# zcash/halo2

Hardware: AMD Instinct MI355X
Metric: Pallas MSM Mscalar-mults/s (+ Fp NTT Gbutterflies/s) at k=20 (higher is better)
Workload: dtype u256 (8x32-bit Montgomery limbs)

## Files before the change

__graft_entry__.py:

```python
import os
import subprocess
import sys

ROOT = os.path.dirname(os.path.abspath(__file__))
if ROOT not in sys.path:
    sys.path.insert(0, ROOT)


def build() -> None:
    subprocess.check_call(["make", "-C", os.path.join(ROOT, "halo2_amd", "csrc"), "-j8", "all", "ab"])
    subprocess.check_call(["make", "-C", os.path.join(ROOT, "oracle")])
    os.makedirs(os.path.join(ROOT, "build"), exist_ok=True)
    subprocess.check_call(["/opt/rocm/bin/hipcc", "--offload-arch=gfx950", "-O3",
                           os.path.join(ROOT, "tests", "native", "field_check.hip"), os.path.join(ROOT, "oracle", "h2_oracle.c"),
                           "-o", os.path.join(ROOT, "build", "field_check")], stderr=subprocess.DEVNULL)
    subprocess.check_call(["/opt/rocm/bin/hipcc", "--offload-arch=gfx950", "-O3",
                           os.path.join(ROOT, "tests", "native", "h2c_edge_driver.hip"), "-o", os.path.join(ROOT, "build", "h2c_edge_driver")])
    subprocess.check_call(["/opt/rocm/bin/hipcc", "--offload-arch=gfx950", "-O3",
                           os.path.join(ROOT, "tests", "native", "field_edge_driver.hip"), "-o", os.path.join(ROOT, "build", "field_edge_driver")])
    subprocess.check_call(["g++", "-O2", "-std=c++17", os.path.join(ROOT, "tests", "native", "host_mirror_check.cpp"),
                           "-L" + os.path.join(ROOT, "halo2_amd"), "-lhalo2_mi355x", "-L" + os.path.join(ROOT, "oracle"), "-lh2oracle",
                           "-Wl,-rpath,$ORIGIN/../halo2_amd", "-Wl,-rpath,$ORIGIN/../oracle", "-lpthread", "-lm",
                           "-o", os.path.join(ROOT, "build", "host_mirror_check")])
    subprocess.check_call(["g++", "-O2", "-std=c++17", os.path.join(ROOT, "tests", "native", "modinv_check.cpp"), "-o", os.path.join(ROOT, "build", "modinv_check")])
    hb = subprocess.run(["/opt/rocm/bin/hipcc", "-O2", "-std=c++17", os.path.join(ROOT, "bench", "native", "h2bench.cpp"),
                         "-L" + os.path.join(ROOT, "oracle"), "-lh2oracle", "-Wl,-rpath,$ORIGIN/../oracle", "-ldl", "-lpthread",
                         "-o", os.path.join(ROOT, "build", "h2bench")], stdout=subprocess.DEVNULL, stderr=subprocess.PIPE, text=True)
    if hb.returncode != 0:
        print("warning: bench/native/h2bench.cpp did not build (the library and the tests do not need it):\n" + hb.stderr[-2000:], file=sys.stderr)
    import halo2_amd
    halo2_amd.lib()


def smoke() -> None:
    import numpy as np

    import halo2_amd as h
    from halo2_amd import fields
    from oracle import c_oracle as co
    from oracle import pasta

    assert h.lib().h2_init(0) == 0, h.lib().h2_last_error()
    curve, n = h.PALLAS, 1 << 12
    sf = co.field_of_curve(curve, "scalar")
    scal = co.random_field(sf, 1, n)
    bases = co.generate_bases(curve, 2, n)
    got = h.best_multiexp(scal, bases, curve)
    want = co.best_multiexp(curve, scal, bases)
    assert co.jac_to_affine_ints(curve, got) == co.jac_to_affine_ints(curve, want), "MSM parity"
    log_n = 12
    a = co.random_field(h.FP, 3, 1 << log_n)
    omega = fields.scalar_limbs(pasta.omega_for(pasta.P, log_n), h.FP)
    assert np.array_equal(h.best_fft(a.copy(), omega, log_n, h.FP), co.best_fft(h.FP, a, omega, log_n)), "NTT parity"
    params = h.Params.new(h.VESTA, 5)
    vs = co.field_of_curve(h.VESTA, "scalar")
    got_w = co.jac_to_affine_ints(h.VESTA, params.commit_lagrange(np.zeros((32, 4), dtype=np.uint64), h.Blind(field=vs)))
    assert got_w == (0x2bbc94ef7b22aebef24f9a4b0cc1831882548b605171366017d45c3e6fd92075,
                     0x082b801a6e176239943bfb759fb02138f47a5c8cc4aa7fa0af559fde4e3abd97), "reference-pinned commitment"
    params.close()
    print("smoke ok: 2^12 Pallas MSM and 2^12 Fp NTT bit-exact vs oracle; Params.new(5) commits to the reference-pinned point")


if __name__ == "__main__":
    build()
    if len(sys.argv) > 1 and sys.argv[1] == "smoke":
        smoke()
```

halo2_amd/csrc/msm_fold.hip:

```cpp
#include "msm_internal.cuh"

namespace h2 {

static_assert(r256_tree_bytes(kTreeLanes) == (kTreeLanes / kGroup) * 128, "a quad of lanes per point of the 8 x 32 tree");

template <int FB>
__global__ void __launch_bounds__(256) msm_finish_buckets(const u32 *__restrict__ heads, const u32 *__restrict__ starts,
                                                          u32 *__restrict__ buckets, u32 *__restrict__ heavy,
                                                          u32 total_buckets, u32 T, u32 div) {
    H2_LATENCY_STAGE();
    const u32 b = (blockIdx.x * blockDim.x + threadIdx.x) / kGroup;
    if (b >= total_buckets) return;
    const bool lead = (threadIdx.x & (kGroup - 1)) == 0;
    const HeadRange h = bucket_heads<false>(starts, b, total_buckets, T, div);
    if (h.h1 <= h.h0) return;
    if (h.h1 - h.h0 > kHeavy && heavy_park<kGroup>(heavy, b, lead)) return;
    xyzz<FB> acc = xyzz_load<FB>(buckets + 32 * (size_t)b);
    xyzz<FB> nxt = xyzz_load<FB>(heads + 32 * (size_t)h.h0);
    for (u32 t = h.h0; t < h.h1; ++t) {
        xyzz<FB> p = nxt;
        if (t + 1 < h.h1) nxt = xyzz_load<FB>(heads + 32 * (size_t)(t + 1));
        xyzz_add_wide<FB>(acc, p);
    }
    if (lead) xyzz_store<FB>(buckets + 32 * (size_t)b, acc);
}
template <int FB>
__global__ void __launch_bounds__(256) msm_finish_heavy(const u32 *__restrict__ heads, const u32 *__restrict__ starts,
                                                        u32 *__restrict__ scratch, const u32 *__restrict__ heavy,
                                                        u32 total_buckets, u32 T, u32 div) {
    H2_LATENCY_STAGE();
    extern __shared__ __attribute__((aligned(16))) u32 sh[];
    if (blockIdx.y >= min(heavy[1], kMaxHeavy)) return;
    const HeadRange h = bucket_heads<false>(starts, heavy[2 + blockIdx.y], total_buckets, T, div);
    const u32 share = (h.h1 - h.h0 + kHeavyBlocks - 1) / kHeavyBlocks;
    const u32 lo = h.h0 + blockIdx.x * share, hi = min(h.h1, lo + share);
    const xyzz<FB> acc = r256_quad_gather<FB>(heads, hi > lo ? hi - lo : 0u, [lo](u32 k) { return lo + k; });
    r256_quads_sum<FB>(acc, sh, blockDim.x / kGroup);
    if (threadIdx.x == 0) {
        xyzz<FB> r = xyzz_load<FB>(sh);
        xyzz_store<FB>(scratch + 32 * ((size_t)blockIdx.y * kHeavyBlocks + blockIdx.x), r);
    }
}
template <int FB>
__global__ void __launch_bounds__(64) msm_finish_heavy2(const u32 *__restrict__ scratch, u32 *__restrict__ buckets,
                                                        const u32 *__restrict__ heavy) {
    H2_LATENCY_STAGE();
    __shared__ __attribute__((aligned(16))) u32 sh[32 * 16];
    if (blockIdx.x >= min(heavy[1], kMaxHeavy)) return;
    const u32 b = heavy[2 + blockIdx.x], q = threadIdx.x / kGroup;
    const bool lead = (threadIdx.x & (kGroup - 1)) == 0;
    const u32 *src = scratch + 32 * ((size_t)blockIdx.x * kHeavyBlocks);
    xyzz<FB> acc = xyzz_load<FB>(src + 32 * q);
    for (u32 i = q + 16; i < kHeavyBlocks; i += 16) {
        xyzz<FB> p = xyzz_load<FB>(src + 32 * i);
        xyzz_add_wide<FB>(acc, p);
    }
    r256_quads_sum<FB>(acc, sh, 16);
    if (q == 0) {
        xyzz<FB> r = xyzz_load<FB>(sh), own = xyzz_load<FB>(buckets + 32 * (size_t)b);
        xyzz_add_wide<FB>(r, own);
        if (lead) xyzz_store<FB>(buckets + 32 * (size_t)b, r);
    }
}

template <int FB>
__global__ void __launch_bounds__(256) msm_bucket_add(u32 *__restrict__ total, const u32 *__restrict__ part, u32 nb) {
    H2_LATENCY_STAGE();
    const u32 b = (blockIdx.x * blockDim.x + threadIdx.x) / kGroup;
    if (b >= nb) return;
    const xyzz<FB> p = xyzz_load<FB>(part + 32 * (size_t)b);
    if (fe_is_zero(p.zz)) return;
    xyzz<FB> acc = xyzz_load<FB>(total + 32 * (size_t)b);
    xyzz_add_wide<FB>(acc, p);
    if ((threadIdx.x & (kGroup - 1)) == 0) xyzz_store<FB>(total + 32 * (size_t)b, acc);
}

template <int FB>
__global__ void __launch_bounds__(256) fold9_finish(const u32 *__restrict__ heads9, const u32 *__restrict__ starts, u32 *__restrict__ buckets9,
                                                    u32 *__restrict__ heavy, u32 total_buckets, u32 T, u32 div, ColStride cs) {
    fold9_stage(cs);
    const u32 b = blockIdx.x * blockDim.x + threadIdx.x;
    if (b >= total_buckets) return;
    if (gridDim.z > 1) {
        heads9 = H2_COLZ(heads9, cs.heads);
        starts = H2_COLZ(starts, cs.starts);
        buckets9 = H2_COLZ(buckets9, cs.buckets);
        heavy = H2_COLZ(heavy, cs.heavy);
    }
    const HeadRange h = bucket_heads<true>(starts, b, total_buckets, T, div);
    if (h.h1 <= h.h0) return;
    if (h.h1 - h.h0 > kHeavy && heavy_park<1>(heavy, b, true)) return;
    xyzz9<FB> acc = xyzz9_load_raw<FB>(buckets9 + 36 * (size_t)b);
    for (u32 t = h.h0; t < h.h1; ++t) xyzz9_add<FB>(acc, xyzz9_load_raw<FB>(heads9 + 36 * (size_t)t));
    xyzz9_store_raw<FB>(buckets9 + 36 * (size_t)b, acc);
}
template <int FB>
__global__ void __launch_bounds__(256, 3) fold9_finish_heavy(const u32 *__restrict__ heads9, const u32 *__restrict__ starts, u32 *__restrict__ scratch9,
                                                          const u32 *__restrict__ heavy, u32 total_buckets, u32 T, u32 div, ColStride cs) {
    fold9_stage(cs);
    __shared__ __attribute__((aligned(16))) u32 sh[32 * 36];
    if (gridDim.z > 1) {
        heavy = H2_COLZ(heavy, cs.heavy);
        heads9 = H2_COLZ(heads9, cs.heads);
        starts = H2_COLZ(starts, cs.starts);
        scratch9 = H2_COLZ(scratch9, cs.hscratch);
    }
    const u32 count = min(heavy[1], kMaxHeavy);
    const HeadSplit hs = head_split<true>(starts, total_buckets, T, div);
    for (u32 slot = blockIdx.y; slot < count; slot += gridDim.y) {
        const HeadRange h = bucket_heads(hs, starts, heavy[2 + slot]);
        const u32 share = (h.h1 - h.h0 + kHeavyBlocks - 1) / kHeavyBlocks;
        const u32 lo = h.h0 + blockIdx.x * share, hi = min(h.h1, lo + share);
        xyzz9<FB> acc = fold9_quad_gather<FB, H2_FOLD_D>(heads9, hi > lo ? hi - lo : 0u, [lo](u32 k) { return lo + k; });
        acc = fold9_quads_sum<FB>(acc, sh);
        if (fold9_root() && (threadIdx.x & (kGroup - 1)) == 0) xyzz9_store_raw<FB>(scratch9 + 36 * ((size_t)slot * kHeavyBlocks + blockIdx.x), acc);
        __syncthreads();
    }
}
template <int FB>
__global__ void __launch_bounds__(64, 3) fold9_finish_heavy2(const u32 *__restrict__ scratch9, u32 *__restrict__ buckets9, const u32 *__restrict__ heavy,
                                                             ColStride cs) {
    fold9_stage(cs);
    __shared__ __attribute__((aligned(16))) u32 sh[8 * 36];
    if (gridDim.z > 1) {
        heavy = H2_COLZ(heavy, cs.heavy);
        scratch9 = H2_COLZ(scratch9, cs.hscratch);
        buckets9 = H2_COLZ(buckets9, cs.buckets);
    }
    const u32 count = min(heavy[1], kMaxHeavy);
    for (u32 slot = blockIdx.x; slot < count; slot += gridDim.x) {
        const u32 b = heavy[2 + slot];
        const u32 *src = scratch9 + 36 * ((size_t)slot * kHeavyBlocks);
        xyzz9<FB> acc = fold9_quad_gather<FB, H2_FOLD_D>(src, kHeavyBlocks, [](u32 k) { return k; });
        acc = fold9_quads_sum<FB>(acc, sh);
        if (fold9_root()) {
            xyzz9_add_wide<FB>(acc, xyzz9_load_raw<FB>(buckets9 + 36 * (size_t)b));
            if ((threadIdx.x & (kGroup - 1)) == 0) xyzz9_store_raw<FB>(buckets9 + 36 * (size_t)b, acc);
        }
        __syncthreads();
    }
}
template <int FB>
__global__ void __launch_bounds__(256, 3) fold9_rowcol(const u32 *__restrict__ buckets9, u32 *__restrict__ lines9, u32 S, u32 NR, ColStride cs) {
    fold9_stage(cs);
    __shared__ __attribute__((aligned(16))) u32 sh[32 * 36];
    if (gridDim.z > 1) {
        buckets9 = H2_COLZ(buckets9, cs.buckets);
        lines9 = H2_COLZ(lines9, cs.lines);
    }
    const bool is_col = blockIdx.x < S;
    const u32 id = is_col ? blockIdx.x : blockIdx.x - S + 1;
    const u32 cnt = is_col ? NR : S;
    const u32 base = blockIdx.y * S * NR + (is_col ? id : id * S), step = is_col ? S : 1;
    xyzz9<FB> acc = fold9_quad_gather<FB, H2_FOLD_D>(buckets9, cnt, [base, step](u32 k) { return base + k * step; });
    acc = fold9_quads_sum<FB>(acc, sh);
    if (fold9_root() && (threadIdx.x & (kGroup - 1)) == 0)
        xyzz9_store_raw<FB>(lines9 + 36 * ((size_t)blockIdx.y * (S + NR) + (is_col ? id : S + id)), acc);
}
template <int FB>
__global__ void __launch_bounds__(256, 3) fold9_planes(const u32 *__restrict__ lines9, u32 *__restrict__ planes9, u32 *__restrict__ counter, u32 S, u32 NR,
                                                    int cb, u32 *__restrict__ out, int out_kind, int out_mont, ColOut co, ColStride cs) {
    fold9_stage(cs);
    __shared__ __attribute__((aligned(16))) u32 sh[32 * 36];
    __shared__ u32 s_last;
    if (gridDim.z > 1) {
        lines9 = H2_COLZ(lines9, cs.lines);
        planes9 = H2_COLZ(planes9, cs.planes);
        counter = H2_COLZ(counter, cs.ctr);
        out = co.out[blockIdx.z];
    }
    const u32 t = blockIdx.x, planes = gridDim.x;
    lines9 += 36 * (size_t)blockIdx.y * (S + NR);
    planes9 += 36 * (size_t)blockIdx.y * 32;
    counter += blockIdx.y;
    out += (out_kind == kOutSliceSum ? 32 : point_out_words(out_kind)) * (size_t)blockIdx.y;
    xyzz9<FB> acc = fold9_quad_gather<FB, H2_FOLD_D>(lines9, fold9_plane_cols(S, cb, t) + fold9_plane_rows(NR, cb, t),
                                                     [=](u32 k) { return fold9_plane_line(S, cb, t, k); });
    acc = fold9_quads_sum<FB>(acc, sh);
    if (!fold9_plane_arrive<FB>(acc, t, planes9, counter, planes, s_last)) return;
    acc = fold9_quad_gather<FB, H2_FOLD_D>(planes9, planes, [](u32 k) { return k; });
    acc = fold9_quads_sum<FB>(acc, sh);
    if (!fold9_root()) return;
    const xyzz<FB> r = xyzz9_to_r256_wide<FB>(acc);
    if ((threadIdx.x & (kGroup - 1)) != 0) return;
    *counter = 0;
    if (out_kind == kOutSliceSum) {
        xyzz_store<FB>(out, r);
        return;
    }
    point_out_store<FB>(out, r, out_kind, out_mont);
}


template <int FB>
__global__ void __launch_bounds__(256) msm_reduce_segments(const u32 *__restrict__ buckets, u32 *__restrict__ partial,
                                                           u32 NB, u32 total_segments, int seg) {
    H2_LATENCY_STAGE();
    const u32 t = (blockIdx.x * blockDim.x + threadIdx.x) / kGroup;
    if (t >= total_segments) return;
    u32 segs_per_slice = NB / seg;
    u32 sl = t / segs_per_slice, sg = t % segs_per_slice;
    const u32 *base = buckets + 32 * ((size_t)sl * NB + (size_t)sg * seg);
    xyzz<FB> run = xyzz_identity<FB>(), acc = xyzz_identity<FB>();
    for (int j = seg - 1; j >= 0; --j) {
        xyzz<FB> bk = xyzz_load<FB>(base + 32 * j);
        xyzz_add_wide<FB>(run, bk);
        xyzz_add_wide<FB>(acc, run);
    }
    xyzz<FB> sh = xyzz_mul_small_wide<FB>(run, sg * seg);
    xyzz_add_wide<FB>(acc, sh);
    if ((threadIdx.x & (kGroup - 1)) == 0) xyzz_store<FB>(partial + 32 * (size_t)t, acc);
}

template <int FB>
__global__ void __launch_bounds__(256) msm_sum_slice(const u32 *__restrict__ partial, u32 *__restrict__ out, u32 per_slice,
                                                     u32 share) {
    H2_LATENCY_STAGE();
    extern __shared__ __attribute__((aligned(16))) u32 sh[];
    const u32 sl = blockIdx.y, blk = blockIdx.x;
    const u32 lo = blk * share, hi = min(per_slice, lo + share);
    const xyzz<FB> acc = r256_quad_gather<FB>(partial + 32 * (size_t)sl * per_slice, hi > lo ? hi - lo : 0u, [lo](u32 k) { return lo + k; });
    r256_quads_sum<FB>(acc, sh, blockDim.x / kGroup);
    if (threadIdx.x == 0) {
        xyzz<FB> r = xyzz_load<FB>(sh);
        xyzz_store<FB>(out + 32 * ((size_t)sl * gridDim.x + blk), r);
    }
}

template <int FB>
__global__ void __launch_bounds__(256) msm_rowcol_sums(const u32 *__restrict__ buckets, u32 *__restrict__ wide, u32 S, u32 NR) {
    H2_LATENCY_STAGE();
    extern __shared__ __attribute__((aligned(16))) u32 sh[];
    const bool is_col = blockIdx.x < S;
    const u32 id = is_col ? blockIdx.x : blockIdx.x - S + 1;
    const size_t base = is_col ? id : (size_t)id * S, step = is_col ? S : 1;
    const xyzz<FB> acc = r256_quad_gather<FB>(buckets, is_col ? NR : S, [base, step](u32 k) { return base + (size_t)k * step; });
    r256_quads_sum<FB>(acc, sh, blockDim.x / kGroup);
    if (threadIdx.x == 0) {
        xyzz<FB> r = xyzz_load<FB>(sh);
        xyzz_store<FB>(wide + 32 * (is_col ? (size_t)id : (size_t)NR + id - 1), r);
    }
}

template <int FB>
__global__ void __launch_bounds__(64) msm_combine(const u32 *__restrict__ slice_sums, int slices, int c, u32 *__restrict__ out,
                                                  int out_kind, int out_mont, int extra_dbl, const u32 *__restrict__ addend, int addend_first) {
    H2_LATENCY_STAGE();
    if (threadIdx.x >= kGroup) return;
    if (gridDim.x > 1) {
        slice_sums += 32 * (size_t)blockIdx.x;
        out += point_out_words(out_kind) * (size_t)blockIdx.x;
        slices = 1;
    }
    xyzz9<FB> r9 = xyzz9_identity<FB>();
    for (int w = slices - 1; w >= 0; --w) {
        if (w != slices - 1)
            for (int k = 0; k < c; ++k) r9 = xyzz9_dbl_wide<FB>(r9);
        const xyzz9<FB> s9 = xyzz9_from_r256_wide<FB>(xyzz_load<FB>(slice_sums + 32 * (size_t)w));
        xyzz9_add_wide<FB>(r9, s9);
    }
    if (addend && addend_first) xyzz9_add_wide<FB>(r9, xyzz9_from_r256_wide<FB>(xyzz_load<FB>(addend)));
    for (int k = 0; k < extra_dbl; ++k) r9 = xyzz9_dbl_wide<FB>(r9);
    if (addend && !addend_first) xyzz9_add_wide<FB>(r9, xyzz9_from_r256_wide<FB>(xyzz_load<FB>(addend)));
    const xyzz<FB> r = xyzz9_to_r256_wide<FB>(r9);
    if (threadIdx.x != 0) return;
    if (out_kind == kOutSliceSum) {
        xyzz_store<FB>(out, r);
        return;
    }
    point_out_store<FB>(out, r, out_kind, out_mont);
}

template <int FB>
__global__ void __launch_bounds__(64) msm_combine_ranges(RangeSums rs, int ranges, int slices, int c, u32 *__restrict__ out, int out_kind, int out_mont) {
    H2_LATENCY_STAGE();
    __shared__ __attribute__((aligned(16))) u32 sh[16 * 36];
    const int w = threadIdx.x / kGroup;
    const bool lead = (threadIdx.x & (kGroup - 1)) == 0;
    if (w < slices) {
        xyzz9<FB> acc = xyzz9_identity<FB>();
        for (int q = 0; q < ranges; ++q) xyzz9_add_wide<FB>(acc, xyzz9_from_r256_wide<FB>(xyzz_load<FB>(rs.p[q] + 32 * (size_t)w)));
        if (lead) xyzz9_store_raw<FB>(sh + 36 * w, acc);
    }
    __syncthreads();
    if (threadIdx.x >= kGroup) return;
    xyzz9<FB> r9 = xyzz9_identity<FB>();
    for (int s = slices - 1; s >= 0; --s) {
        if (s != slices - 1)
            for (int k = 0; k < c; ++k) r9 = xyzz9_dbl_wide<FB>(r9);
        xyzz9_add_wide<FB>(r9, xyzz9_load_raw<FB>(sh + 36 * s));
    }
    const xyzz<FB> r = xyzz9_to_r256_wide<FB>(r9);
    if (threadIdx.x == 0) point_out_store<FB>(out, r, out_kind, out_mont);
}

#define H2_FOLD_FB(fb, f, ...) ((fb) == FP ? f<FP>(__VA_ARGS__) : f<FQ>(__VA_ARGS__))

template <int FB> static void fold9_group_launch(hipStream_t st, const Fold9Group &g) {
    const ColStride &cs = g.cs;
    const u32 fz = cs.joined ? 1 : g.cols, ftb = cs.joined ? g.cols * g.tb : g.tb;
    const u32 S = g.wideS, NR = g.wideNR;
    u32 *lines = g.lines9 + 36 * (size_t)g.slice0 * (S + NR);
    hipLaunchKernelGGL((fold9_finish<FB>), dim3((ftb + 255) / 256, 1, fz), dim3(256), 0, st, g.heads9, g.starts, g.buckets9, g.heavy, ftb, g.T, g.lane_div, cs);
    hipLaunchKernelGGL((fold9_finish_heavy<FB>), dim3(kHeavyBlocks, kHeavyRows, fz), dim3(256), 0, st, g.heads9, g.starts, g.hscratch, (const u32 *)g.heavy, ftb, g.T, g.lane_div, cs);
    hipLaunchKernelGGL((fold9_finish_heavy2<FB>), dim3(kHeavyRows, 1, fz), dim3(64), 0, st, (const u32 *)g.hscratch, g.buckets9, (const u32 *)g.heavy, cs);
    hipLaunchKernelGGL((fold9_rowcol<FB>), dim3(S + NR - 1, g.nslices, g.cols), dim3(256), 0, st, (const u32 *)g.buckets9, lines, S, NR, cs);
    hipLaunchKernelGGL((fold9_planes<FB>), dim3(fold9_plane_count(g.c), g.nslices, g.cols), dim3(256), 0, st, (const u32 *)lines, g.planes9 + 36 * (size_t)g.slice0 * 32, g.ctr + g.slice0, S, NR,
                       fold9_col_bits(S), g.out + 32 * (size_t)g.slice0, g.out_kind, g.out_mont ? 1 : 0, g.co, cs);
}
void fold9_group(int fb, hipStream_t st, const Fold9Group &g) { H2_FOLD_FB(fb, fold9_group_launch, st, g); }

template <int FB> static void combine_launch(hipStream_t st, size_t lds, u32 outputs, const u32 *slice_sums, int slices, int c, u32 *out, int out_kind, bool out_mont,
                                             int extra_dbl, const u32 *addend, bool addend_first) {
    hipLaunchKernelGGL((msm_combine<FB>), dim3(outputs), dim3(64), lds, st, slice_sums, slices, c, out, out_kind, out_mont ? 1 : 0, extra_dbl, addend, addend_first ? 1 : 0);
}
void msm_combine_launch(int fb, hipStream_t st, size_t lds, u32 outputs, const u32 *slice_sums, int slices, int c, u32 *out, int out_kind, bool out_mont,
                        int extra_dbl, const u32 *addend, bool addend_first) {
    H2_FOLD_FB(fb, combine_launch, st, lds, outputs, slice_sums, slices, c, out, out_kind, out_mont, extra_dbl, addend, addend_first);
}
int msm_combine_allow_lds(size_t bytes) {
    H2_HIP(hipFuncSetAttribute((const void *)msm_combine<FP>, hipFuncAttributeMaxDynamicSharedMemorySize, (int)bytes));
    H2_HIP(hipFuncSetAttribute((const void *)msm_combine<FQ>, hipFuncAttributeMaxDynamicSharedMemorySize, (int)bytes));
    return H2_OK;
}
template <int FB> static void combine_ranges_launch(hipStream_t st, const RangeSums &rs, int ranges, int slices, int c, u32 *out, int out_kind, bool out_mont) {
    hipLaunchKernelGGL((msm_combine_ranges<FB>), dim3(1), dim3(64), 0, st, rs, ranges, slices, c, out, out_kind, out_mont ? 1 : 0);
}
void msm_combine_ranges_launch(int fb, hipStream_t st, const RangeSums &rs, int ranges, int slices, int c, u32 *out, int out_kind, bool out_mont) {
    H2_FOLD_FB(fb, combine_ranges_launch, st, rs, ranges, slices, c, out, out_kind, out_mont);
}
template <int FB> static void bucket_add_launch(hipStream_t st, u32 *total, const u32 *part, u32 nb) {
    hipLaunchKernelGGL((msm_bucket_add<FB>), dim3((nb * kGroup + 255) / 256), dim3(256), 0, st, total, part, nb);
}
void msm_bucket_add_launch(int fb, hipStream_t st, u32 *total, const u32 *part, u32 nb) { H2_FOLD_FB(fb, bucket_add_launch, st, total, part, nb); }

template <int FB> static int fold_r256_launch(MsmContext &cx, const MsmPlan &p, const MsmArgs &a, hipStream_t st) {
    const u32 tb = p.tb, T = p.T;
    const size_t tree_lds = r256_tree_bytes(kTreeLanes);
    if (!p.fold_only) {
        hipLaunchKernelGGL((msm_finish_buckets<FB>), dim3((tb * kGroup + 255) / 256), dim3(256), 0, st, cx.heads.as<u32>(),
                           cx.starts.as<u32>(), cx.buckets.as<u32>(), cx.heavy.as<u32>(), tb, T, p.lane_div);
        hipLaunchKernelGGL((msm_finish_heavy<FB>), dim3(kHeavyBlocks, kMaxHeavy), dim3(kTreeLanes), tree_lds, st,
                           cx.heads.as<u32>(), cx.starts.as<u32>(), cx.hscratch.as<u32>(), cx.heavy.as<u32>(), tb, T, p.lane_div);
        hipLaunchKernelGGL((msm_finish_heavy2<FB>), dim3(kMaxHeavy), dim3(64), 0, st, cx.hscratch.as<u32>(), cx.buckets.as<u32>(), cx.heavy.as<u32>());
    }
    if (p.add_only) {
        bucket_add_launch<FB>(st, a.add_into, cx.buckets.as<u32>(), tb);
        return H2_OK;
    }
    const R256Fold f = r256_fold_geometry(p.sh, p.wide_reduce, p.wideNR);
    const u32 *fold_src = p.fold_only ? a.fold_from : cx.buckets.as<u32>();
    if (p.wide_reduce) {
        u32 *wide = cx.partial.as<u32>() + 32 * (size_t)(2 * p.wideNR / kSeg);
        H2_HIP(hipMemsetAsync(wide, 0, (size_t)2 * p.wideNR * 128, st));
        hipLaunchKernelGGL((msm_rowcol_sums<FB>), dim3(p.wideS + p.wideNR - 1), dim3(kTreeLanes), tree_lds, st, fold_src, wide, p.wideS, p.wideNR);
        fold_src = wide;
    }
    hipLaunchKernelGGL((msm_reduce_segments<FB>), dim3((f.segs * kGroup + 255) / 256), dim3(256), 0, st, fold_src, cx.partial.as<u32>(), f.nb, f.segs, f.seg);
    for (int l = 0; l < f.levels; ++l) {
        const R256Fold::Level &v = f.level[l];
        hipLaunchKernelGGL((msm_sum_slice<FB>), dim3(v.blocks, f.slices), dim3(kTreeLanes), tree_lds, st, l ? cx.heads.as<u32>() : cx.partial.as<u32>(),
                           l == f.levels - 1 ? cx.ssums.as<u32>() : cx.heads.as<u32>(), v.per_slice, v.share);
    }
    combine_launch<FB>(st, 0, p.pair ? 2 : 1, cx.ssums.as<u32>(), (int)f.slices, f.c, (u32 *)a.d_out, a.out_kind, a.form == H2_FORM_MONTGOMERY, 0, nullptr, false);
    return H2_OK;
}
int fold_r256(int fb, MsmContext &cx, const MsmPlan &p, const MsmArgs &a, hipStream_t st) { return H2_FOLD_FB(fb, fold_r256_launch, cx, p, a, st); }

}
```

Baseline: 1143.

## Run final MSM window combine on a full wavefront with row-parallel limb arithmetic

Replaces the serial kGroup-lane Horner combine (doublings and adds across window slices) with a 64-lane version. Each 16-lane DPP row holds one coordinate's 9 limbs, and each field multiply is spread across limbs using row broadcast and row shift. Point doubling and addition run their four multiplies at once across the four rows and exchange results with ds_bpermute. This targets the latency of the tail combine kernel, which runs on a single wave. It adds cross-lane traffic and a new, complex carry-normalisation path that must stay bit-exact.

Measured after the change: 1144, median of 6. Within noise of the previous version (+0.1%).

```diff
diff --git a/__graft_entry__.py b/__graft_entry__.py
--- a/__graft_entry__.py
+++ b/__graft_entry__.py
@@ -18,6 +18,8 @@
                            os.path.join(ROOT, "tests", "native", "h2c_edge_driver.hip"), "-o", os.path.join(ROOT, "build", "h2c_edge_driver")])
     subprocess.check_call(["/opt/rocm/bin/hipcc", "--offload-arch=gfx950", "-O3",
                            os.path.join(ROOT, "tests", "native", "field_edge_driver.hip"), "-o", os.path.join(ROOT, "build", "field_edge_driver")])
+    subprocess.check_call(["/opt/rocm/bin/hipcc", "--offload-arch=gfx950", "-O3", "-std=c++17",
+                           os.path.join(ROOT, "tests", "native", "row_point_driver.hip"), "-o", os.path.join(ROOT, "build", "row_point_driver")])
     subprocess.check_call(["g++", "-O2", "-std=c++17", os.path.join(ROOT, "tests", "native", "host_mirror_check.cpp"),
                            "-L" + os.path.join(ROOT, "halo2_amd"), "-lhalo2_mi355x", "-L" + os.path.join(ROOT, "oracle"), "-lh2oracle",
                            "-Wl,-rpath,$ORIGIN/../halo2_amd", "-Wl,-rpath,$ORIGIN/../oracle", "-lpthread", "-lm",
diff --git a/halo2_amd/csrc/curve9_row.cuh b/halo2_amd/csrc/curve9_row.cuh
--- /dev/null
+++ b/halo2_amd/csrc/curve9_row.cuh
@@ -0,0 +1,200 @@
+#pragma once
+#include "curve9.cuh"
+
+namespace h2 {
+
+static constexpr int kDppRowShl = 0x100, kDppRowShr = 0x110, kDppRowRor = 0x120, kDppRowBcast = 0x150;
+
+template <int CTRL> __device__ __forceinline__ i32 row_dpp(i32 x) {
+    return __builtin_amdgcn_update_dpp(0, x, CTRL, 0xf, 0xf, true);
+}
+template <int N> __device__ __forceinline__ i32 row_bcast(i32 x) { return row_dpp<kDppRowBcast + N>(x); }
+template <int N> __device__ __forceinline__ i32 row_shr(i32 x) {
+    if constexpr (N == 0) return x;
+    else return row_dpp<kDppRowShr + N>(x);
+}
+template <int CTRL> __device__ __forceinline__ i64 row_dpp64(i64 x) {
+    const u32 lo = (u32)row_dpp<CTRL>((i32)(u32)x), hi = (u32)row_dpp<CTRL>((i32)(u32)((unsigned long long)x >> 32));
+    return (i64)(((unsigned long long)hi << 32) | lo);
+}
+
+struct fe9r {
+    i32 v;
+};
+__device__ __forceinline__ int row_lane() { return threadIdx.x & 15; }
+__device__ __forceinline__ int row_index() { return (threadIdx.x >> 4) & 3; }
+
+template <int F> struct RowCtx {
+    int j;
+    i32 p;
+    u32 nm;
+    unsigned long long bias;
+};
+template <int F> __device__ __forceinline__ RowCtx<F> row_ctx() {
+    RowCtx<F> c;
+    const int j = row_lane();
+    c.j = j;
+    c.p = j == 0 ? 1 : j == 1 ? Mod9<F>::P1 : j == 2 ? Mod9<F>::P2 : j == 3 ? Mod9<F>::P3 : j == 4 ? Mod9<F>::P4 : j == 8 ? P9_8 : 0;
+    c.nm = j < 8 ? M29 : ~0u;
+    const unsigned long long top = 1ull << 63, back = 1ull << 34;
+    c.bias = (j < 8 ? top : 0ull) - (j >= 1 && j < 9 ? back : 0ull) - (j < 7 ? (unsigned long long)M29 : 0ull);
+    return c;
+}
+
+__device__ __forceinline__ fe9r fe9r_add(fe9r a, fe9r b) { return fe9r{a.v + b.v}; }
+__device__ __forceinline__ fe9r fe9r_sub(fe9r a, fe9r b) { return fe9r{a.v - b.v}; }
+__device__ __forceinline__ fe9r fe9r_dbl(fe9r a) { return fe9r{a.v << 1}; }
+template <int F> __device__ __forceinline__ fe9r fe9r_norm(const RowCtx<F> &c, fe9r a) {
+    const i32 carry = c.j < 8 ? a.v >> 29 : 0;
+    return fe9r{(i32)(((u32)a.v & c.nm) + (u32)row_dpp<kDppRowShr + 1>(carry))};
+}
+template <int F> __device__ __forceinline__ fe9r fe9r_quadruple_norm(const RowCtx<F> &c, fe9r a) {
+    const u32 t = (u32)a.v << 2;
+    const i32 carry = c.j < 8 ? (i32)(t >> 29) : 0;
+    return fe9r{(i32)((t & c.nm) + (u32)row_dpp<kDppRowShr + 1>(carry))};
+}
+
+template <int F> __device__ __forceinline__ fe9r fe9r_mul(const RowCtx<F> &c, fe9r a, fe9r b) {
+    i64 V = (i64)M29;
+#define H2_ROW_TERM(I) V += (i64)row_bcast<I>(a.v) * row_shr<I>(b.v);
+    H2_ROW_TERM(0) H2_ROW_TERM(1) H2_ROW_TERM(2) H2_ROW_TERM(3) H2_ROW_TERM(4) H2_ROW_TERM(5) H2_ROW_TERM(6) H2_ROW_TERM(7) H2_ROW_TERM(8)
+#undef H2_ROW_TERM
+    i64 X = (i64)row_bcast<8>(a.v) * row_dpp<kDppRowRor + 8>(b.v);
+    i64 carry = 0;
+    i32 mk;
+#define H2_ROW_STEP(K)                                                        \
+    {                                                                         \
+        const i64 t = K ? V + row_dpp64<kDppRowShr + 1>(carry) : V;           \
+        carry = t >> 29;                                                      \
+        mk = row_bcast<K>((i32)(~(u32)t & M29));                              \
+        V += (i64)mk * row_shr<K>(c.p);                                       \
+    }
+    H2_ROW_STEP(0) H2_ROW_STEP(1) H2_ROW_STEP(2) H2_ROW_STEP(3) H2_ROW_STEP(4) H2_ROW_STEP(5) H2_ROW_STEP(6) H2_ROW_STEP(7) H2_ROW_STEP(8)
+#undef H2_ROW_STEP
+    X += (i64)mk * P9_8;
+    const i64 c9 = row_dpp64<kDppRowShr + 1>(carry);
+    i64 R = c.j >= 9 ? V + (c.j == 9 ? c9 : (i64)0) : (c.j == 0 ? X : (i64)0);
+    R = row_dpp64<kDppRowRor + 7>(R);
+    unsigned long long u = (unsigned long long)R + c.bias;
+    const unsigned long long h1 = c.j < 8 ? u >> 29 : 0ull;
+    const unsigned long long keep = c.j < 8 ? (unsigned long long)M29 : ~0ull;
+    u = (u & keep) + (unsigned long long)row_dpp64<kDppRowShr + 1>((i64)h1);
+    const u32 h2 = c.j < 8 ? (u32)(u >> 29) : 0u;
+    u32 w = ((u32)u & c.nm) + (u32)row_dpp<kDppRowShr + 1>((i32)h2);
+    const u32 h3 = c.j < 8 ? w >> 29 : 0u;
+    w = (w & c.nm) + (u32)row_dpp<kDppRowShr + 1>((i32)h3);
+    return fe9r{(i32)w};
+}
+
+__device__ __forceinline__ fe9r fe9r_spread(int j, const fe9 &a) {
+    i32 v = 0;
+#pragma unroll
+    for (int i = 0; i < 9; i++) v = j == i ? a.v[i] : v;
+    return fe9r{v};
+}
+__device__ __forceinline__ fe9 fe9r_collect(fe9r a) {
+    fe9 r;
+    r.v[0] = row_bcast<0>(a.v); r.v[1] = row_bcast<1>(a.v); r.v[2] = row_bcast<2>(a.v);
+    r.v[3] = row_bcast<3>(a.v); r.v[4] = row_bcast<4>(a.v); r.v[5] = row_bcast<5>(a.v);
+    r.v[6] = row_bcast<6>(a.v); r.v[7] = row_bcast<7>(a.v); r.v[8] = row_bcast<8>(a.v);
+    return r;
+}
+
+template <int SRC> __device__ __forceinline__ fe9r row_from(int j, fe9r a) { return fe9r{__builtin_amdgcn_ds_bpermute((SRC * 16 + j) << 2, a.v)}; }
+__device__ __forceinline__ fe9r row_sel(int r, fe9r a0, fe9r a1, fe9r a2, fe9r a3) {
+    return fe9r{r == 0 ? a0.v : r == 1 ? a1.v : r == 2 ? a2.v : a3.v};
+}
+
+template <int F> struct xyzz9r {
+    fe9r x, y, zz, zzz;
+};
+template <int F> __device__ __forceinline__ xyzz9r<F> xyzz9r_identity() { return xyzz9r<F>{fe9r{0}, fe9r{0}, fe9r{0}, fe9r{0}}; }
+template <int F> __device__ __forceinline__ bool xyzz9r_is_identity(const xyzz9r<F> &p) { return __builtin_amdgcn_ballot_w64(p.zz.v != 0) == 0; }
+
+template <int F> __device__ __forceinline__ xyzz9<F> xyzz9r_collect(const xyzz9r<F> &p) {
+    return xyzz9<F>{fe9r_collect(p.x), fe9r_collect(p.y), fe9r_collect(p.zz), fe9r_collect(p.zzz)};
+}
+template <int F> __device__ __forceinline__ xyzz9r<F> xyzz9r_spread(int j, const xyzz9<F> &p) {
+    return xyzz9r<F>{fe9r_spread(j, p.x), fe9r_spread(j, p.y), fe9r_spread(j, p.zz), fe9r_spread(j, p.zzz)};
+}
+
+template <int F> __device__ __forceinline__ xyzz9r<F> xyzz9r_load_raw(const RowCtx<F> &c, const u32 *src) {
+    const u32 *w = src + (c.j < 9 ? c.j : 0);
+    const u32 keep = c.j < 9 ? ~0u : 0u;
+    return xyzz9r<F>{fe9r{(i32)(w[0] & keep)}, fe9r{(i32)(w[9] & keep)}, fe9r{(i32)(w[18] & keep)}, fe9r{(i32)(w[27] & keep)}};
+}
+
+template <int F> __device__ __forceinline__ xyzz9r<F> xyzz9_dbl_row(const RowCtx<F> &c, const xyzz9r<F> &p) {
+    if (xyzz9r_is_identity(p)) return p;
+    const int r = row_index(), j = c.j;
+    const fe9r u = fe9r_dbl(p.y);
+    const fe9r o1 = row_sel(r, p.y, p.x, p.y, p.y);
+    const fe9r r1 = fe9r_mul<F>(c, o1, o1);
+    const fe9r yy = row_from<0>(j, r1), xx = row_from<1>(j, r1);
+    const fe9r v = fe9r_quadruple_norm<F>(c, yy);
+    const fe9r m = fe9r_norm<F>(c, fe9r_add(fe9r_dbl(xx), xx));
+    const fe9r r2 = fe9r_mul<F>(c, row_sel(r, u, p.x, m, v), row_sel(r, v, v, m, p.zz));
+    const fe9r w = row_from<0>(j, r2), s = row_from<1>(j, r2), mm = row_from<2>(j, r2);
+    xyzz9r<F> o;
+    o.zz = row_from<3>(j, r2);
+    o.x = fe9r_norm<F>(c, fe9r_sub(fe9r_sub(mm, s), s));
+    const fe9r r3 = fe9r_mul<F>(c, row_sel(r, m, w, w, w), row_sel(r, fe9r_sub(s, o.x), p.y, p.zzz, p.zzz));
+    o.y = fe9r_norm<F>(c, fe9r_sub(row_from<0>(j, r3), row_from<1>(j, r3)));
+    o.zzz = row_from<2>(j, r3);
+    return o;
+}
+
+template <int F> __device__ __forceinline__ void xyzz9_add_row(const RowCtx<F> &c, xyzz9r<F> &acc, const xyzz9r<F> &q) {
+    if (xyzz9r_is_identity(q)) return;
+    if (xyzz9r_is_identity(acc)) {
+        acc = q;
+        return;
+    }
+    const int r = row_index(), j = c.j;
+    const fe9r r1 = fe9r_mul<F>(c, row_sel(r, acc.x, q.x, acc.y, q.y), row_sel(r, q.zz, acc.zz, q.zzz, acc.zzz));
+    const fe9r u1 = row_from<0>(j, r1), u2 = row_from<1>(j, r1), s1 = row_from<2>(j, r1), s2 = row_from<3>(j, r1);
+    const fe9r p = fe9r_sub(u2, u1), rr = fe9r_sub(s2, s1);
+    if ((((u32)__builtin_amdgcn_readfirstlane(p.v) + 16u) & M29) <= 32u) {
+        xyzz9<F> special;
+        if (xyzz9_add_rare<F>(fe9r_collect(p), fe9r_collect(rr), xyzz9r_collect(q), &special)) {
+            acc = xyzz9r_spread(j, special);
+            return;
+        }
+    }
+    const fe9r r2 = fe9r_mul<F>(c, row_sel(r, p, rr, acc.zz, acc.zzz), row_sel(r, p, rr, q.zz, q.zzz));
+    const fe9r pp = row_from<0>(j, r2), r_sq = row_from<1>(j, r2), za = row_from<2>(j, r2), zb = row_from<3>(j, r2);
+    const fe9r r3 = fe9r_mul<F>(c, row_sel(r, p, u1, za, za), pp);
+    const fe9r ppp = row_from<0>(j, r3), qq = row_from<1>(j, r3);
+    acc.zz = row_from<2>(j, r3);
+    const fe9r x3 = fe9r_norm<F>(c, fe9r_sub(fe9r_sub(r_sq, ppp), fe9r_dbl(qq)));
+    const fe9r r4 = fe9r_mul<F>(c, row_sel(r, rr, s1, zb, zb), row_sel(r, fe9r_sub(qq, x3), ppp, ppp, ppp));
+    acc.x = x3;
+    acc.y = fe9r_norm<F>(c, fe9r_sub(row_from<0>(j, r4), row_from<1>(j, r4)));
+    acc.zzz = row_from<2>(j, r4);
+}
+
+template <int F> __device__ __forceinline__ xyzz9r<F> xyzz9_from_r256_row(const RowCtx<F> &c, const xyzz<F> &p) {
+    if (xyzz_is_identity(p)) return xyzz9r_identity<F>();
+    const int r = row_index(), j = c.j;
+    fe coord;
+#pragma unroll
+    for (int i = 0; i < 8; i++) coord.v[i] = r == 0 ? p.x.v[i] : r == 1 ? p.y.v[i] : r == 2 ? p.zz.v[i] : p.zzz.v[i];
+    const fe9r t = fe9r_mul<F>(c, fe9r_spread(j, fe9_unpack(coord)), fe9r_spread(j, fe9_k_in<F>()));
+    return xyzz9r<F>{row_from<0>(j, t), row_from<1>(j, t), row_from<2>(j, t), row_from<3>(j, t)};
+}
+template <int F> __device__ __forceinline__ xyzz<F> xyzz9_to_r256_row(const RowCtx<F> &c, const xyzz9r<F> &p) {
+    if (xyzz9r_is_identity(p)) return xyzz_identity<F>();
+    const fe9r t = fe9r_mul<F>(c, row_sel(row_index(), p.x, p.y, p.zz, p.zzz), fe9r_spread(c.j, fe9_k_out<F>()));
+    const fe canon = fe9_canonical_small<F>(fe9r_collect(t));
+    xyzz<F> o;
+#pragma unroll
+    for (int i = 0; i < 8; i++) {
+        o.x.v[i] = (u32)__builtin_amdgcn_readlane((int)canon.v[i], 0);
+        o.y.v[i] = (u32)__builtin_amdgcn_readlane((int)canon.v[i], 16);
+        o.zz.v[i] = (u32)__builtin_amdgcn_readlane((int)canon.v[i], 32);
+        o.zzz.v[i] = (u32)__builtin_amdgcn_readlane((int)canon.v[i], 48);
+    }
+    return o;
+}
+
+}
diff --git a/halo2_amd/csrc/msm_fold.hip b/halo2_amd/csrc/msm_fold.hip
--- a/halo2_amd/csrc/msm_fold.hip
+++ b/halo2_amd/csrc/msm_fold.hip
@@ -1,4 +1,5 @@
 #include "msm_internal.cuh"
+#include "curve9_row.cuh"
 
 namespace h2 {
 
@@ -246,23 +247,23 @@
 __global__ void __launch_bounds__(64) msm_combine(const u32 *__restrict__ slice_sums, int slices, int c, u32 *__restrict__ out,
                                                   int out_kind, int out_mont, int extra_dbl, const u32 *__restrict__ addend, int addend_first) {
     H2_LATENCY_STAGE();
-    if (threadIdx.x >= kGroup) return;
     if (gridDim.x > 1) {
         slice_sums += 32 * (size_t)blockIdx.x;
         out += point_out_words(out_kind) * (size_t)blockIdx.x;
         slices = 1;
     }
-    xyzz9<FB> r9 = xyzz9_identity<FB>();
+    const RowCtx<FB> rc = row_ctx<FB>();
+    xyzz9r<FB> r9 = xyzz9r_identity<FB>();
     for (int w = slices - 1; w >= 0; --w) {
         if (w != slices - 1)
-            for (int k = 0; k < c; ++k) r9 = xyzz9_dbl_wide<FB>(r9);
-        const xyzz9<FB> s9 = xyzz9_from_r256_wide<FB>(xyzz_load<FB>(slice_sums + 32 * (size_t)w));
-        xyzz9_add_wide<FB>(r9, s9);
-    }
-    if (addend && addend_first) xyzz9_add_wide<FB>(r9, xyzz9_from_r256_wide<FB>(xyzz_load<FB>(addend)));
-    for (int k = 0; k < extra_dbl; ++k) r9 = xyzz9_dbl_wide<FB>(r9);
-    if (addend && !addend_first) xyzz9_add_wide<FB>(r9, xyzz9_from_r256_wide<FB>(xyzz_load<FB>(addend)));
-    const xyzz<FB> r = xyzz9_to_r256_wide<FB>(r9);
+            for (int k = 0; k < c; ++k) r9 = xyzz9_dbl_row<FB>(rc, r9);
+        const xyzz9r<FB> s9 = xyzz9_from_r256_row<FB>(rc, xyzz_load<FB>(slice_sums + 32 * (size_t)w));
+        xyzz9_add_row<FB>(rc, r9, s9);
+    }
+    if (addend && addend_first) xyzz9_add_row<FB>(rc, r9, xyzz9_from_r256_row<FB>(rc, xyzz_load<FB>(addend)));
+    for (int k = 0; k < extra_dbl; ++k) r9 = xyzz9_dbl_row<FB>(rc, r9);
+    if (addend && !addend_first) xyzz9_add_row<FB>(rc, r9, xyzz9_from_r256_row<FB>(rc, xyzz_load<FB>(addend)));
+    const xyzz<FB> r = xyzz9_to_r256_row<FB>(rc, r9);
     if (threadIdx.x != 0) return;
     if (out_kind == kOutSliceSum) {
         xyzz_store<FB>(out, r);
@@ -283,14 +284,14 @@
         if (lead) xyzz9_store_raw<FB>(sh + 36 * w, acc);
     }
     __syncthreads();
-    if (threadIdx.x >= kGroup) return;
-    xyzz9<FB> r9 = xyzz9_identity<FB>();
+    const RowCtx<FB> rc = row_ctx<FB>();
+    xyzz9r<FB> r9 = xyzz9r_identity<FB>();
     for (int s = slices - 1; s >= 0; --s) {
         if (s != slices - 1)
-            for (int k = 0; k < c; ++k) r9 = xyzz9_dbl_wide<FB>(r9);
-        xyzz9_add_wide<FB>(r9, xyzz9_load_raw<FB>(sh + 36 * s));
-    }
-    const xyzz<FB> r = xyzz9_to_r256_wide<FB>(r9);
+            for (int k = 0; k < c; ++k) r9 = xyzz9_dbl_row<FB>(rc, r9);
+        xyzz9_add_row<FB>(rc, r9, xyzz9r_load_raw<FB>(rc, sh + 36 * s));
+    }
+    const xyzz<FB> r = xyzz9_to_r256_row<FB>(rc, r9);
     if (threadIdx.x == 0) point_out_store<FB>(out, r, out_kind, out_mont);
 }
 
```
